# yjzxkxdn/HubertFA

Hardware: NVIDIA B200
Metric: dp_cells_per_s (higher is better)
Workload: dtype f32

## Files before the change

### hubertfa_b200/csrc/hfa_dp_skew.cu

```cuda
#include <cstdlib>

#include "hfa_common.cuh"

namespace {

__device__ __forceinline__ float sk_lds_f32(uint32_t addr)
{
    float v;
    asm volatile("ld.shared.f32 %0, [%1];" : "=f"(v) : "r"(addr));
    return v;
}
__device__ __forceinline__ float2 sk_lds_f2(uint32_t addr)
{
    float2 v;
    asm volatile("ld.shared.v2.f32 {%0, %1}, [%2];" : "=f"(v.x), "=f"(v.y) : "r"(addr));
    return v;
}
__device__ __forceinline__ void sk_sts_f32(uint32_t addr, float v)
{
    asm volatile("st.shared.f32 [%0], %1;" ::"r"(addr), "f"(v) : "memory");
}
__device__ __forceinline__ int sk_lds_i32(uint32_t addr)
{
    int v;
    asm volatile("ld.shared.s32 %0, [%1];" : "=r"(v) : "r"(addr) : "memory");
    return v;
}
__device__ __forceinline__ void sk_sts_i32(uint32_t addr, int v)
{
    asm volatile("st.shared.s32 [%0], %1;" ::"r"(addr), "r"(v) : "memory");
}
__device__ __forceinline__ void sk_mbar_init(uint32_t bar, uint32_t count)
{
    asm volatile("mbarrier.init.shared::cta.b64 [%0], %1;" ::"r"(bar), "r"(count) : "memory");
}
__device__ __forceinline__ void sk_mbar_expect_tx(uint32_t bar, uint32_t bytes)
{
    asm volatile("mbarrier.arrive.expect_tx.shared::cta.b64 _, [%0], %1;" ::"r"(bar), "r"(bytes) : "memory");
}
__device__ __forceinline__ void sk_mbar_arrive(uint32_t bar)
{
    asm volatile("mbarrier.arrive.shared::cta.b64 _, [%0];" ::"r"(bar) : "memory");
}
__device__ __forceinline__ void sk_mbar_wait(uint32_t bar, uint32_t parity)
{
    uint32_t spins = 0;
    for (;;) {
        uint32_t ok;
        asm volatile(
            "{\n"
            ".reg .pred p;\n"
            "mbarrier.try_wait.parity.shared::cta.b64 p, [%1], %2;\n"
            "selp.u32 %0, 1, 0, p;\n"
            "}\n"
            : "=r"(ok)
            : "r"(bar), "r"(parity)
            : "memory");
        if (ok) return;
        if (++spins > (1u << 24)) __trap();
    }
}
__device__ __forceinline__ void sk_bulk_load(uint32_t dst, const void *src, uint32_t bytes, uint32_t bar)
{
    asm volatile("cp.async.bulk.shared::cta.global.mbarrier::complete_tx::bytes [%0], [%1], %2, [%3];" ::"r"(dst),
                 "l"(src), "r"(bytes), "r"(bar)
                 : "memory");
}
__device__ __forceinline__ void sk_tensor_load_2d(uint32_t dst, const void *tmap, int x, int y, uint32_t bar)
{
    asm volatile(
        "cp.async.bulk.tensor.2d.shared::cta.global.tile.mbarrier::complete_tx::bytes [%0], [%1, {%2, %3}], [%4];" ::"r"(dst),
        "l"(tmap), "r"(x), "r"(y), "r"(bar)
        : "memory");
}
__device__ __forceinline__ void sk_bulk_store(void *dst, uint32_t src, uint32_t bytes)
{
    asm volatile("cp.async.bulk.global.shared::cta.bulk_group [%0], [%1], %2;" ::"l"(dst), "r"(src), "r"(bytes) : "memory");
}
__device__ __forceinline__ bool sk_elect_one()
{
    uint32_t pred;
    asm volatile(
        "{\n"
        ".reg .pred p;\n"
        "elect.sync _|p, 0xffffffff;\n"
        "selp.u32 %0, 1, 0, p;\n"
        "}\n"
        : "=r"(pred));
    return pred != 0;
}
__device__ __forceinline__ void sk_bulk_wait_read_1() { asm volatile("cp.async.bulk.wait_group.read 1;" ::: "memory"); }

__device__ __forceinline__ ulonglong2 sk_ld_slot(const ulonglong2 *p)
{
    ulonglong2 v;
    asm volatile("ld.relaxed.gpu.global.v2.u64 {%0, %1}, [%2];" : "=l"(v.x), "=l"(v.y) : "l"(p) : "memory");
    return v;
}
__device__ __forceinline__ void sk_st_slot(ulonglong2 *p, unsigned long long a, unsigned long long b)
{
    asm volatile("st.relaxed.gpu.global.v2.u64 [%0], {%1, %2};" ::"l"(p), "l"(a), "l"(b) : "memory");
}
__device__ __forceinline__ void sk_st_word(unsigned long long *p, unsigned long long a)
{
    asm volatile("st.relaxed.gpu.global.u64 [%0], %1;" ::"l"(p), "l"(a) : "memory");
}
__device__ __forceinline__ unsigned long long sk_pack(float v, uint32_t tag)
{
    return (unsigned long long)__float_as_uint(v) | ((unsigned long long)tag << 32);
}

__device__ __forceinline__ void sk_select(float up1, float stay, float up2, double pe, uint32_t sp_hi, uint32_t mr,
                                          float &dp, double &P, uint32_t &acc)
{
    asm("{\n\t"
        ".reg .pred q1, q2, q3;\n\t"
        ".reg .f32 m;\n\t"
        ".reg .f64 pn;\n\t"
        ".reg .b32 lo, hi;\n\t"
        "setp.gt.f32 q1, %3, %4;\n\t"
        "max.f32 m, %4, %3;\n\t"
        "setp.gt.f32 q2, %5, m;\n\t"
        "max.f32 %0, m, %5;\n\t"
        "@q1 lop3.b32 %2, %2, %8, 0x0000ffff, 0xf8;\n\t"
        "@q2 lop3.b32 %2, %2, %8, 0xffff0000, 0xf8;\n\t"
        "or.pred q3, q1, q2;\n\t"
        "setp.gt.or.f64 q3, %6, %1, q3;\n\t"
        "selp.f64 pn, %6, %1, q3;\n\t"
        "mov.b64 {lo, hi}, pn;\n\t"
        "and.b32 hi, hi, %7;\n\t"
        "mov.b64 %1, {lo, hi};\n\t"
        "}"
        : "=&f"(dp), "+d"(P), "+r"(acc)
        : "f"(up1), "f"(stay), "f"(up2), "d"(pe), "r"(sp_hi), "r"(mr));
}
__device__ __forceinline__ void sk_select_guarded(float up1, float stay, float up2, double pe, uint32_t sp_hi,
                                                  uint32_t mr, int live, float &dp, double &P, uint32_t &acc)
{
    asm("{\n\t"
        ".reg .pred pl, q1, q2, q3;\n\t"
        ".reg .f32 m, dn;\n\t"
        ".reg .f64 pn;\n\t"
        ".reg .b32 lo, hi, msk;\n\t"
        "setp.ne.b32 pl, %9, 0;\n\t"
        "setp.gt.and.f32 q1, %3, %4, pl;\n\t"
        "max.f32 m, %4, %3;\n\t"
        "setp.gt.and.f32 q2, %5, m, pl;\n\t"
        "max.f32 dn, m, %5;\n\t"
        "selp.f32 %0, dn, %0, pl;\n\t"
        "@q1 lop3.b32 %2, %2, %8, 0x0000ffff, 0xf8;\n\t"
        "@q2 lop3.b32 %2, %2, %8, 0xffff0000, 0xf8;\n\t"
        "or.pred q3, q1, q2;\n\t"
        "setp.gt.or.f64 q3, %6, %1, q3;\n\t"
        "and.pred q3, q3, pl;\n\t"
        "selp.f64 pn, %6, %1, q3;\n\t"
        "mov.b64 {lo, hi}, pn;\n\t"
        "selp.b32 msk, %7, 0xffffffff, pl;\n\t"
        "and.b32 hi, hi, msk;\n\t"
        "mov.b64 %1, {lo, hi};\n\t"
        "}"
        : "+f"(dp), "+d"(P), "+r"(acc)
        : "f"(up1), "f"(stay), "f"(up2), "d"(pe), "r"(sp_hi), "r"(mr), "r"(live));
}

constexpr int SK_BOXW = HFA_SKEW_BOX;
constexpr int BLK = HFA_SKEW_BLK;
constexpr uint32_t SK_ROW_B = SK_BOXW * 4u;
constexpr uint32_t SK_STG_B = BLK * SK_ROW_B;
constexpr uint32_t SK_EDGE_B = BLK * 8u;
constexpr uint32_t SK_DPST_B = BLK * 128u;
constexpr uint32_t SK_PUB_B = (2 * BLK + BLK + 32) * 4u;
constexpr int SK_LOOK = 3;
static_assert(BLK == 16 || BLK == 32, "a block is one or two backpointer words long");

template <int NSTG> struct SkSmem {
    static constexpr uint32_t TILE = 0;
    static constexpr uint32_t EDGE = TILE + (NSTG + 1) * SK_STG_B;
    static constexpr uint32_t DPST = EDGE + (NSTG + 1) * SK_EDGE_B;
    static constexpr uint32_t PUB = DPST + 2 * SK_DPST_B;
    static constexpr uint32_t FULL = PUB + 2 * SK_PUB_B;
    static constexpr uint32_t SLOT = FULL + NSTG * 8;
    static constexpr uint32_t BYTES = SLOT + 16;
};

template <int D, int NSTG, bool KEEP, bool DUMP>
__global__ void __launch_bounds__(32)
hfa_dp_skew_kernel(HfaWs ws, int item_begin, int32_t *ticket, float *__restrict__ dp_dump, int force_slow)
{
    using SM = SkSmem<NSTG>;
    constexpr int R = NSTG * BLK;
    constexpr int Q = (31 * D + BLK - 1) / BLK;
    constexpr int PF = NSTG - 1 - Q;
    static_assert(D >= 2, "advance scores must be at least two iterations old when they are consumed");
    static_assert(PF >= 1, "ring too small for this skew");
    extern __shared__ __align__(128) unsigned char smem_raw[];
    uint32_t sm0;
    {
        const uint32_t a = hfa_smem_u32(smem_raw);
        asm volatile("mov.u32 %0, %1;" : "=r"(sm0) : "r"(a));
    }

    const int lane = threadIdx.x;
    if (lane == 0) {
        sk_sts_i32(sm0 + SM::SLOT, (int)atomicInc(reinterpret_cast<unsigned int *>(ticket), gridDim.x - 1));
#pragma unroll
        for (int s = 0; s < NSTG; ++s) sk_mbar_init(sm0 + SM::FULL + 8u * s, 1);
        hfa_fence_mbar_init();
    }
    __syncwarp();
    const int item = item_begin + sk_lds_i32(sm0 + SM::SLOT);
    const HfaBandItem bi = ws.band_items[item];
    const int u = bi.utt, w = bi.band;
    const HfaUtt m = ws.utt[u];
    const int T = m.T, S = m.S, Sp = m.Sp;
    const bool has_left = w > 0, has_right = w + 1 < hfa_skew_strips(Sp);
    const int c0 = HFA_SKEW_OWN * w;
    const int s = c0 + lane;
    const bool ghost = has_left && lane < 2;
    const bool real = !ghost && s < Sp;
    const int NB = hfa_skew_blocks(D, T);
    const int n_rows = (T + 15) >> 4;
    const float2 *g_edge = ws.edge2 + m.edge_off;
    uint32_t *g_bp = ws.bp + m.bp_off;
    const unsigned char *tmap = static_cast<const unsigned char *>(ws.tmaps) + (size_t)m.tmap * 128;
    const double ratio = __ddiv_rn((double)T, (double)S);
    const float NEG = HFA_NEG_INF, POS = __uint_as_float(0x7f800000u);

    const int32_t *ids = ws.ids + m.seg_off;
    uint32_t sp_hi = 0xffffffffu;
    float jcap = NEG;
    if (s < S) {
        if (ids[s] == 0) sp_hi = 0u;
        if (s >= 2 && ids[s - 1] == 0) jcap = POS;
    }
    const bool lead_sp = (ids[0] == 0) && (S > 1);
    const bool seeded = !ghost && (s == 0 || (s == 1 && lead_sp));
    const float cap1 = (s == 0) ? NEG : POS;

    const int edge_len = (T + 15) & ~15;
    auto issue = [&](int i, int st) {
        const int t0 = i * BLK;
        const uint32_t bar = sm0 + SM::FULL + 8u * (uint32_t)st;
        if (t0 >= T) {
            sk_mbar_arrive(bar);
            return;
        }
        const uint32_t ebytes = (uint32_t)min(BLK, edge_len - t0) * 8u;
        const uint32_t bytes = SK_STG_B + ebytes;
        sk_mbar_expect_tx(bar, st == 0 ? 2u * bytes : bytes);
        sk_tensor_load_2d(sm0 + SM::TILE + (uint32_t)st * SK_STG_B, tmap, c0 & ~3, t0, bar);
        sk_bulk_load(sm0 + SM::EDGE + (uint32_t)st * SK_EDGE_B, g_edge + t0, ebytes, bar);
        if (st == 0) {
            sk_tensor_load_2d(sm0 + SM::TILE + (uint32_t)NSTG * SK_STG_B, tmap, c0 & ~3, t0, bar);
            sk_bulk_load(sm0 + SM::EDGE + (uint32_t)NSTG * SK_EDGE_B, g_edge + t0, ebytes, bar);
        }
    };
    static_assert(PF + 1 <= NSTG, "prologue fills distinct stages");
    if (sk_elect_one())
        for (int i = 0; i <= PF && i < NB; ++i) issue(i, i);
    int st_issue = (PF + 1) % NSTG;
    int st_wait = 0;
    uint32_t par_wait = 0;

    float dp = NEG;
    double P = __longlong_as_double(0xfff0000000000000ll);
    uint32_t bits = 0;
    float q1[D], q2[2 * D];
#pragma unroll
    for (int i = 0; i < D; ++i) q1[i] = NEG;
#pragma unroll
    for (int i = 0; i < 2 * D; ++i) q2[i] = NEG;

    int u_row = ((-lane * D) % R + R) % R;
    const uint32_t tile_sa = sm0 + SM::TILE + 4u * (uint32_t)(lane + (c0 & 3));
    const uint32_t edge_sa = sm0 + SM::EDGE;
    const uint32_t dpst_sa = sm0 + SM::DPST + 4u * (uint32_t)lane;
    const int o_res = (lane * D) & 15;
    const int q_rows = (lane * D + 15) >> 4;
    const uint32_t m16 = o_res ? ((0xffffu << (16 - o_res)) & 0xffffu) : 0xffffu;
    const uint32_t hi_mask = m16 | (m16 << 16);
    const uint32_t mrot0 = 0x00010001u << ((16 - o_res) & 15);
    const ulonglong2 *left_x = reinterpret_cast<const ulonglong2 *>(ws.band_xchg) +
                               (has_left ? ws.band_items[item - 1].xoff : 0);
    ulonglong2 *my_x = reinterpret_cast<ulonglong2 *>(ws.band_xchg) + bi.xoff;
    const uint32_t pub_sa = sm0 + SM::PUB +
                            ((has_right && lane == 31) ? 0u : (has_right && lane == 30) ? 4u * BLK
                                                                                        : 8u * BLK + 4u * (uint32_t)lane);
    uint32_t *bp_ptr = g_bp + (int64_t)(-q_rows) * Sp + s;
    int bp_row = -q_rows;
    float *g_dp = (KEEP && m.dp_off >= 0) ? ws.dp_store + m.dp_off + (int64_t)w * NB * (BLK * 32) : nullptr;

    ulonglong2 xv_next = make_ulonglong2(0ull, 0ull);
    auto slot_needed = [&](int jj) { const int t = BLK * jj + lane; return has_left && lane < BLK && t >= 1 && t < T; };
    if (slot_needed(0)) xv_next = sk_ld_slot(left_x + lane);

    auto flush_bits = [&](uint32_t acc, bool all_valid) {
        if (real && (all_valid || (bp_row >= 0 && bp_row < n_rows))) *bp_ptr = bits | (acc & hi_mask);
        bits = acc & ~hi_mask;
        bp_ptr += Sp;
        ++bp_row;
    };

    for (int j = 0; j < NB; ++j) {
        sk_mbar_wait(sm0 + SM::FULL + 8u * (uint32_t)st_wait, par_wait);
        const int st_cur = st_wait;
        if (++st_wait == NSTG) {
            st_wait = 0;
            par_wait ^= 1u;
        }

        if (has_left) {
            const int t = BLK * j + lane;
            const bool need = slot_needed(j);
            ulonglong2 *src = const_cast<ulonglong2 *>(left_x) + t;
            const uint32_t tag = (uint32_t)t + 1u;
            ulonglong2 v = xv_next;
            uint32_t spins = 0;
            for (;;) {
                const bool ok = !need || ((uint32_t)(v.x >> 32) == tag && (uint32_t)(v.y >> 32) == tag);
                if (__all_sync(0xffffffffu, ok)) break;
                if (++spins > (1u << 26)) __trap();
                if (!ok) v = sk_ld_slot(src);
            }
            if (slot_needed(j + 1)) xv_next = sk_ld_slot(src + BLK);
            if (lane < BLK) {
                const float a30 = need ? __uint_as_float((uint32_t)v.y) : 0.0f;
                const float a31 = need ? __uint_as_float((uint32_t)v.x) : 0.0f;
                const uint32_t row_sa = sm0 + SM::TILE + (uint32_t)st_cur * SK_STG_B + (uint32_t)lane * SK_ROW_B +
                                        4u * (uint32_t)(c0 & 3);
                sk_sts_f32(row_sa, a30);
                sk_sts_f32(row_sa + 4u, a31);
                if (st_cur == 0) {
                    sk_sts_f32(row_sa + (uint32_t)NSTG * SK_STG_B, a30);
                    sk_sts_f32(row_sa + (uint32_t)NSTG * SK_STG_B + 4u, a31);
                }
                if (need) sk_st_slot(src, 0ull, 0ull);
            }
            hfa_fence_async_smem();
            __syncwarp();
        }
        const uint32_t e_sa = tile_sa + (uint32_t)u_row * SK_ROW_B;
        const uint32_t d_sa = edge_sa + (uint32_t)u_row * 8u;
        const uint32_t k_sa = dpst_sa + (uint32_t)(j & 1) * SK_DPST_B;
        const uint32_t p_sa = pub_sa + (uint32_t)(j & 1) * SK_PUB_B;
        const bool steady = (BLK * j - 31 * D >= 1) && (BLK * j + BLK - 1 <= T - 1);

        if ((j == 0 && !has_left) || force_slow) {
            uint32_t acc = 0;
#pragma unroll 1
            for (int k = 0; k < BLK; ++k) {
                const int t = BLK * j + k - lane * D;
                const bool live = (t >= 1) && (t < T);
                const float e = sk_lds_f32(e_sa + SK_ROW_B * k);
                const float2 ed = sk_lds_f2(d_sa + 8u * k);
                const float base = __fadd_rn(dp, e);
                const float stay = __fadd_rn(base, ed.y);
                const float adv = __double2float_rn(__dadd_rn((double)__fadd_rn(base, ed.x), P));
                const float advx = ghost ? e : adv;
                const float n1 = fminf(__shfl_up_sync(0xffffffffu, advx, 1), cap1);
                const float n2 = fminf(__shfl_up_sync(0xffffffffu, advx, 2), jcap);
                const float up1 = q1[0], up2 = q2[0];
#pragma unroll
                for (int i = 0; i + 1 < D; ++i) q1[i] = q1[i + 1];
                q1[D - 1] = n1;
#pragma unroll
                for (int i = 0; i + 1 < 2 * D; ++i) q2[i] = q2[i + 1];
                q2[2 * D - 1] = n2;
                sk_sts_f32(p_sa + 4u * k, advx);
                const float mm = fmaxf(stay, up1);
                const bool b1 = up1 > stay, b2 = up2 > mm;
                const double pe = __dmul_rn((double)e, ratio);
                if (live) {
                    dp = fmaxf(mm, up2);
                    if (b1) acc |= 1u << (t & 15);
                    if (b2) acc |= 0x10000u << (t & 15);
                    const double pn = (b1 || b2 || pe > P) ? pe : P;
                    P = __hiloint2double(__double2hiint(pn) & (int)sp_hi, __double2loint(pn));
                }
                if (t == 0 && seeded) {
                    dp = e;
                    P = pe;
                }
                if (KEEP) sk_sts_f32(k_sa + 128u * k, dp);
                if (DUMP) {
                    if (!ghost && s < S && t >= 0 && t < T) dp_dump[m.cell_off + (int64_t)t * S + s] = dp;
                }
                if ((k & 15) == 15) {
                    flush_bits(acc, false);
                    acc = 0;
                }
            }
        } else {
            float ev[BLK];
            float2 dv[BLK];
#pragma unroll
            for (int k = 0; k < SK_LOOK; ++k) {
                ev[k] = sk_lds_f32(e_sa + SK_ROW_B * k);
                dv[k] = sk_lds_f2(d_sa + 8u * k);
            }
            float r1[BLK + D], r2[BLK + 2 * D];
#pragma unroll
            for (int i = 0; i < D; ++i) r1[i] = q1[i];
#pragma unroll
            for (int i = 0; i < 2 * D; ++i) r2[i] = q2[i];
            uint32_t mr = mrot0, acc = 0;
            if (!DUMP && steady) {
#pragma unroll
                for (int k = 0; k < BLK; ++k) {
                    if (k + SK_LOOK < BLK) {
                        ev[k + SK_LOOK] = sk_lds_f32(e_sa + SK_ROW_B * (k + SK_LOOK));
                        dv[k + SK_LOOK] = sk_lds_f2(d_sa + 8u * (k + SK_LOOK));
                    }
                    const float e = ev[k];
                    const float base = __fadd_rn(dp, e);
                    const float stay = __fadd_rn(base, dv[k].y);
                    const float adv = __double2float_rn(__dadd_rn((double)__fadd_rn(base, dv[k].x), P));
                    const float advx = ghost ? e : adv;
                    r1[k + D] = fminf(__shfl_up_sync(0xffffffffu, advx, 1), cap1);
                    r2[k + 2 * D] = fminf(__shfl_up_sync(0xffffffffu, advx, 2), jcap);
                    sk_sts_f32(p_sa + 4u * k, advx);
                    const double pe = __dmul_rn((double)e, ratio);
                    sk_select(r1[k], stay, r2[k], pe, sp_hi, mr, dp, P, acc);
                    mr = __funnelshift_l(mr, mr, 1);
                    if (KEEP) sk_sts_f32(k_sa + 128u * k, dp);
                    if ((k & 15) == 15) {
                        flush_bits(acc, true);
                        acc = 0;
                    }
                }
            } else {
                const int tb = BLK * j - lane * D - 1;
#pragma unroll
                for (int k = 0; k < BLK; ++k) {
                    if (k + SK_LOOK < BLK) {
                        ev[k + SK_LOOK] = sk_lds_f32(e_sa + SK_ROW_B * (k + SK_LOOK));
                        dv[k + SK_LOOK] = sk_lds_f2(d_sa + 8u * (k + SK_LOOK));
                    }
                    const int live = (unsigned)(tb + k) < (unsigned)(T - 1);
                    const float e = ev[k];
                    const float base = __fadd_rn(dp, e);
                    const float stay = __fadd_rn(base, dv[k].y);
                    const float adv = __double2float_rn(__dadd_rn((double)__fadd_rn(base, dv[k].x), P));
                    const float advx = ghost ? e : adv;
                    r1[k + D] = fminf(__shfl_up_sync(0xffffffffu, advx, 1), cap1);
                    r2[k + 2 * D] = fminf(__shfl_up_sync(0xffffffffu, advx, 2), jcap);
                    sk_sts_f32(p_sa + 4u * k, advx);
                    const double pe = __dmul_rn((double)e, ratio);
                    sk_select_guarded(r1[k], stay, r2[k], pe, sp_hi, mr, live, dp, P, acc);
                    mr = __funnelshift_l(mr, mr, 1);
                    if (KEEP) sk_sts_f32(k_sa + 128u * k, dp);
                    if (DUMP) {
                        const int t = tb + 1 + k;
                        if (!ghost && s < S && t >= 0 && t < T) dp_dump[m.cell_off + (int64_t)t * S + s] = dp;
                    }
                    if ((k & 15) == 15) {
                        flush_bits(acc, false);
                        acc = 0;
                    }
                }
            }
#pragma unroll
            for (int i = 0; i < D; ++i) q1[i] = r1[BLK + i];
#pragma unroll
            for (int i = 0; i < 2 * D; ++i) q2[i] = r2[BLK + i];
        }
        if (KEEP) hfa_fence_async_smem();
        __syncwarp();
        if (has_right) {
#pragma unroll
            for (int q = lane; q < 2 * BLK; q += 32) {
                const int half = q / BLK, i = q % BLK;
                const int t = BLK * j + i - (31 - half) * D;
                if (steady || (t >= 1 && t < T))
                    sk_st_word(reinterpret_cast<unsigned long long *>(my_x + t) + half,
                               sk_pack(sk_lds_f32(sm0 + SM::PUB + (uint32_t)(j & 1) * SK_PUB_B + 4u * (uint32_t)q),
                                       (uint32_t)t + 1u));
            }
        }
        if (sk_elect_one()) {
            if (KEEP && g_dp != nullptr) {
                sk_bulk_store(g_dp + (int64_t)j * (BLK * 32), sm0 + SM::DPST + (uint32_t)(j & 1) * SK_DPST_B, SK_DPST_B);
                hfa_bulk_commit();
                sk_bulk_wait_read_1();
            }
            if (j + PF + 1 < NB) issue(j + PF + 1, st_issue);
        }
        if (++st_issue == NSTG) st_issue = 0;
        u_row += BLK;
        if (u_row >= R) u_row -= R;
    }
    if (real && o_res != 0 && bp_row >= 0 && bp_row < n_rows) *bp_ptr = bits;
    if (!ghost) {
        if (s == S - 1) ws.dp_last[2 * u] = dp;
        if (s == S - 2) ws.dp_last[2 * u + 1] = dp;
    }
    if (KEEP && sk_elect_one()) hfa_bulk_wait_all();
}

template <int D, int NSTG, bool KEEP, bool DUMP>
cudaError_t launch_skew(const HfaLaunchCtx &c, int item_begin, int n_items, int32_t *ticket, float *dp_dump,
                        int force_slow)
{
    const size_t smem = SkSmem<NSTG>::BYTES;
    cudaError_t e = cudaFuncSetAttribute(hfa_dp_skew_kernel<D, NSTG, KEEP, DUMP>,
                                         cudaFuncAttributeMaxDynamicSharedMemorySize, (int)smem);
    if (e != cudaSuccess) return e;
    hfa_dp_skew_kernel<D, NSTG, KEEP, DUMP><<<n_items, 32, smem, c.stream>>>(c.ws, item_begin, ticket, dp_dump,
                                                                            force_slow);
    return cudaGetLastError();
}

template <int D, int NSTG>
cudaError_t launch_skew_d(const HfaLaunchCtx &c, int item_begin, int n_items, int32_t *ticket, bool keep_dp,
                          float *dp_dump, int force_slow)
{
    if (dp_dump != nullptr)
        return keep_dp ? launch_skew<D, NSTG, true, true>(c, item_begin, n_items, ticket, dp_dump, force_slow)
                       : launch_skew<D, NSTG, false, true>(c, item_begin, n_items, ticket, dp_dump, force_slow);
    return keep_dp ? launch_skew<D, NSTG, true, false>(c, item_begin, n_items, ticket, dp_dump, force_slow)
                   : launch_skew<D, NSTG, false, false>(c, item_begin, n_items, ticket, dp_dump, force_slow);
}

}

cudaError_t hfa_launch_dp_skew(const HfaLaunchCtx &c, int d, int item_begin, int n_items, int32_t *ticket,
                               bool keep_dp, float *dp_dump)
{
    if (n_items <= 0) return cudaSuccess;
    if (c.ws.tmaps == nullptr) return cudaErrorNotSupported;
    const char *sl = getenv("HFA_SKEW_SLOW");
    const int force_slow = (sl && sl[0] == '1') ? 1 : 0;
    constexpr int NS = HFA_SKEW_BLK == 32 ? 5 : 12;
    if (d == 2) return launch_skew_d<2, NS>(c, item_begin, n_items, ticket, keep_dp, dp_dump, force_slow);
    if (d == 3) return launch_skew_d<3, NS>(c, item_begin, n_items, ticket, keep_dp, dp_dump, force_slow);
    return cudaErrorInvalidValue;
}
```

Measured before the change: 84.63 billion.

## Split DP skew kernel into producer and consumer warps with mbarrier handoff

Adds a second warp per block that handles TMA issue, the left-neighbour exchange polling, publishing of boundary scores to the right band, and bulk stores of DP tiles. The compute warp now only waits on a READY barrier and signals DONE, with publish/store buffers tripled so the producer can lag. This aims to take the serialized exchange spin and store and issue latency off the DP critical path. In exchange it doubles the threads per block and adds barrier traffic, and the warp-slot parity trick used to pick the producer role is fragile.

Measured after the change: 87.57 billion, median of 6. +3.5%, better.

```diff
diff --git a/hubertfa_b200/csrc/hfa_dp_skew.cu b/hubertfa_b200/csrc/hfa_dp_skew.cu
--- a/hubertfa_b200/csrc/hfa_dp_skew.cu
+++ b/hubertfa_b200/csrc/hfa_dp_skew.cu
@@ -42,7 +42,7 @@
 {
     asm volatile("mbarrier.arrive.shared::cta.b64 _, [%0];" ::"r"(bar) : "memory");
 }
-__device__ __forceinline__ void sk_mbar_wait(uint32_t bar, uint32_t parity)
+__device__ __forceinline__ void sk_mbar_wait(uint32_t bar, uint32_t parity, uint32_t limit)
 {
     uint32_t spins = 0;
     for (;;) {
@@ -57,8 +57,22 @@
             : "r"(bar), "r"(parity)
             : "memory");
         if (ok) return;
-        if (++spins > (1u << 24)) __trap();
+        if (++spins > limit) __trap();
     }
+}
+__device__ __forceinline__ bool sk_mbar_test(uint32_t bar, uint32_t parity)
+{
+    uint32_t ok;
+    asm volatile(
+        "{\n"
+        ".reg .pred p;\n"
+        "mbarrier.test_wait.parity.shared::cta.b64 p, [%1], %2;\n"
+        "selp.u32 %0, 1, 0, p;\n"
+        "}\n"
+        : "=r"(ok)
+        : "r"(bar), "r"(parity)
+        : "memory");
+    return ok != 0;
 }
 __device__ __forceinline__ void sk_bulk_load(uint32_t dst, const void *src, uint32_t bytes, uint32_t bar)
 {
@@ -90,6 +104,7 @@
     return pred != 0;
 }
 __device__ __forceinline__ void sk_bulk_wait_read_1() { asm volatile("cp.async.bulk.wait_group.read 1;" ::: "memory"); }
+__device__ __forceinline__ void sk_bulk_wait_read_0() { asm volatile("cp.async.bulk.wait_group.read 0;" ::: "memory"); }
 
 __device__ __forceinline__ ulonglong2 sk_ld_slot(const ulonglong2 *p)
 {
@@ -171,20 +186,23 @@
 constexpr uint32_t SK_DPST_B = BLK * 128u;
 constexpr uint32_t SK_PUB_B = (2 * BLK + BLK + 32) * 4u;
 constexpr int SK_LOOK = 3;
+constexpr int SK_NBUF = 3;
 static_assert(BLK == 16 || BLK == 32, "a block is one or two backpointer words long");
 
 template <int NSTG> struct SkSmem {
     static constexpr uint32_t TILE = 0;
     static constexpr uint32_t EDGE = TILE + (NSTG + 1) * SK_STG_B;
     static constexpr uint32_t DPST = EDGE + (NSTG + 1) * SK_EDGE_B;
-    static constexpr uint32_t PUB = DPST + 2 * SK_DPST_B;
-    static constexpr uint32_t FULL = PUB + 2 * SK_PUB_B;
-    static constexpr uint32_t SLOT = FULL + NSTG * 8;
+    static constexpr uint32_t PUB = DPST + SK_NBUF * SK_DPST_B;
+    static constexpr uint32_t FULL = PUB + SK_NBUF * SK_PUB_B;
+    static constexpr uint32_t READY = FULL + NSTG * 8;
+    static constexpr uint32_t DONE = READY + NSTG * 8;
+    static constexpr uint32_t SLOT = DONE + NSTG * 8;
     static constexpr uint32_t BYTES = SLOT + 16;
 };
 
 template <int D, int NSTG, bool KEEP, bool DUMP>
-__global__ void __launch_bounds__(32)
+__global__ void __launch_bounds__(64)
 hfa_dp_skew_kernel(HfaWs ws, int item_begin, int32_t *ticket, float *__restrict__ dp_dump, int force_slow)
 {
     using SM = SkSmem<NSTG>;
@@ -200,14 +218,23 @@
         asm volatile("mov.u32 %0, %1;" : "=r"(sm0) : "r"(a));
     }
 
-    const int lane = threadIdx.x;
-    if (lane == 0) {
+    if (threadIdx.x == 0) {
+        unsigned hw_slot;
+        asm volatile("mov.u32 %0, %%warpid;" : "=r"(hw_slot));
+        sk_sts_i32(sm0 + SM::SLOT + 4u, (int)((hw_slot >> 2) & 1u));
         sk_sts_i32(sm0 + SM::SLOT, (int)atomicInc(reinterpret_cast<unsigned int *>(ticket), gridDim.x - 1));
 #pragma unroll
-        for (int s = 0; s < NSTG; ++s) sk_mbar_init(sm0 + SM::FULL + 8u * s, 1);
+        for (int s = 0; s < NSTG; ++s) {
+            sk_mbar_init(sm0 + SM::FULL + 8u * s, 1);
+            sk_mbar_init(sm0 + SM::READY + 8u * s, 32);
+            sk_mbar_init(sm0 + SM::DONE + 8u * s, 32);
+        }
         hfa_fence_mbar_init();
     }
-    __syncwarp();
+    __syncthreads();
+    const int lane = threadIdx.x & 31;
+    const bool producer =
+        __shfl_sync(0xffffffffu, (threadIdx.x >> 5) ^ (unsigned)sk_lds_i32(sm0 + SM::SLOT + 4u), 0) != 0;
     const int item = item_begin + sk_lds_i32(sm0 + SM::SLOT);
     const HfaBandItem bi = ws.band_items[item];
     const int u = bi.utt, w = bi.band;
@@ -215,14 +242,135 @@
     const int T = m.T, S = m.S, Sp = m.Sp;
     const bool has_left = w > 0, has_right = w + 1 < hfa_skew_strips(Sp);
     const int c0 = HFA_SKEW_OWN * w;
+    const int NB = hfa_skew_blocks(D, T);
+
+    if (producer) {
+        const float2 *g_edge = ws.edge2 + m.edge_off;
+        const unsigned char *tmap = static_cast<const unsigned char *>(ws.tmaps) + (size_t)m.tmap * 128;
+        float *g_dp = (KEEP && m.dp_off >= 0) ? ws.dp_store + m.dp_off + (int64_t)w * NB * (BLK * 32) : nullptr;
+        const int edge_len = (T + 15) & ~15;
+        auto issue = [&](int i, int st) {
+            const int t0 = i * BLK;
+            const uint32_t bar = sm0 + SM::FULL + 8u * (uint32_t)st;
+            if (t0 >= T) {
+                sk_mbar_arrive(bar);
+                return;
+            }
+            const uint32_t ebytes = (uint32_t)min(BLK, edge_len - t0) * 8u;
+            const uint32_t bytes = SK_STG_B + ebytes;
+            sk_mbar_expect_tx(bar, st == 0 ? 2u * bytes : bytes);
+            sk_tensor_load_2d(sm0 + SM::TILE + (uint32_t)st * SK_STG_B, tmap, c0 & ~3, t0, bar);
+            sk_bulk_load(sm0 + SM::EDGE + (uint32_t)st * SK_EDGE_B, g_edge + t0, ebytes, bar);
+            if (st == 0) {
+                sk_tensor_load_2d(sm0 + SM::TILE + (uint32_t)NSTG * SK_STG_B, tmap, c0 & ~3, t0, bar);
+                sk_bulk_load(sm0 + SM::EDGE + (uint32_t)NSTG * SK_EDGE_B, g_edge + t0, ebytes, bar);
+            }
+        };
+        static_assert(PF + 1 <= NSTG, "prologue fills distinct stages");
+        if (sk_elect_one())
+            for (int i = 0; i <= PF && i < NB; ++i) issue(i, i);
+
+        const ulonglong2 *left_x = reinterpret_cast<const ulonglong2 *>(ws.band_xchg) +
+                                   (has_left ? ws.band_items[item - 1].xoff : 0);
+        ulonglong2 *my_x = reinterpret_cast<ulonglong2 *>(ws.band_xchg) + bi.xoff;
+        auto slot_needed = [&](int jj) { const int t = BLK * jj + lane; return has_left && lane < BLK && t >= 1 && t < T; };
+        ulonglong2 xv = make_ulonglong2(0ull, 0ull);
+        if (slot_needed(0)) xv = sk_ld_slot(left_x + lane);
+
+        int a = 0, st_a = 0, buf_b = 0;
+        uint32_t par_a = 0;
+        int b = 0, st_b = 0;
+        uint32_t par_b = 0;
+        int st_issue = (PF + 1) % NSTG;
+        uint32_t spins = 0;
+        while (b < NB) {
+            if (b < a && __all_sync(0xffffffffu, sk_mbar_test(sm0 + SM::DONE + 8u * (uint32_t)st_b, par_b))) {
+                if (has_right) {
+#pragma unroll
+                    for (int q = lane; q < 2 * BLK; q += 32) {
+                        const int half = q / BLK, i = q % BLK;
+                        const int t = BLK * b + i - (31 - half) * D;
+                        if (t >= 1 && t < T)
+                            sk_st_word(reinterpret_cast<unsigned long long *>(my_x + t) + half,
+                                       sk_pack(sk_lds_f32(sm0 + SM::PUB + (uint32_t)buf_b * SK_PUB_B + 4u * (uint32_t)q),
+                                               (uint32_t)t + 1u));
+                    }
+                }
+                if (sk_elect_one()) {
+                    if (KEEP && g_dp != nullptr) {
+                        sk_bulk_store(g_dp + (int64_t)b * (BLK * 32), sm0 + SM::DPST + (uint32_t)buf_b * SK_DPST_B,
+                                      SK_DPST_B);
+                        hfa_bulk_commit();
+                    }
+                    if (b + PF + 1 < NB) issue(b + PF + 1, st_issue);
+                }
+                if (++st_issue == NSTG) st_issue = 0;
+                if (++st_b == NSTG) {
+                    st_b = 0;
+                    par_b ^= 1u;
+                }
+                if (++buf_b == SK_NBUF) buf_b = 0;
+                ++b;
+                spins = 0;
+                continue;
+            }
+            if (a < NB && a <= b + SK_NBUF - 1 &&
+                __all_sync(0xffffffffu, sk_mbar_test(sm0 + SM::FULL + 8u * (uint32_t)st_a, par_a))) {
+                bool go = true;
+                if (has_left) {
+                    const int t = BLK * a + lane;
+                    const bool need = slot_needed(a);
+                    ulonglong2 *src = const_cast<ulonglong2 *>(left_x) + t;
+                    const uint32_t tag = (uint32_t)t + 1u;
+                    const bool ok = !need || ((uint32_t)(xv.x >> 32) == tag && (uint32_t)(xv.y >> 32) == tag);
+                    go = __all_sync(0xffffffffu, ok);
+                    if (!go) {
+                        if (!ok) xv = sk_ld_slot(src);
+                    } else {
+                        const ulonglong2 v = xv;
+                        xv = slot_needed(a + 1) ? sk_ld_slot(src + BLK) : make_ulonglong2(0ull, 0ull);
+                        if (lane < BLK) {
+                            const float a30 = need ? __uint_as_float((uint32_t)v.y) : 0.0f;
+                            const float a31 = need ? __uint_as_float((uint32_t)v.x) : 0.0f;
+                            const uint32_t row_sa = sm0 + SM::TILE + (uint32_t)st_a * SK_STG_B + (uint32_t)lane * SK_ROW_B +
+                                                    4u * (uint32_t)(c0 & 3);
+                            sk_sts_f32(row_sa, a30);
+                            sk_sts_f32(row_sa + 4u, a31);
+                            if (st_a == 0) {
+                                sk_sts_f32(row_sa + (uint32_t)NSTG * SK_STG_B, a30);
+                                sk_sts_f32(row_sa + (uint32_t)NSTG * SK_STG_B + 4u, a31);
+                            }
+                            if (need) sk_st_slot(src, 0ull, 0ull);
+                        }
+                        hfa_fence_async_smem();
+                    }
+                }
+                if (go) {
+                    if (KEEP && a >= SK_NBUF && sk_elect_one()) {
+                        if (a == b + SK_NBUF - 1) sk_bulk_wait_read_0();
+                        else sk_bulk_wait_read_1();
+                    }
+                    sk_mbar_arrive(sm0 + SM::READY + 8u * (uint32_t)st_a);
+                    if (++st_a == NSTG) {
+                        st_a = 0;
+                        par_a ^= 1u;
+                    }
+                    ++a;
+                    spins = 0;
+                    continue;
+                }
+            }
+            if (++spins > (1u << 26)) __trap();
+        }
+        if (KEEP && sk_elect_one()) hfa_bulk_wait_all();
+        return;
+    }
+
     const int s = c0 + lane;
     const bool ghost = has_left && lane < 2;
     const bool real = !ghost && s < Sp;
-    const int NB = hfa_skew_blocks(D, T);
     const int n_rows = (T + 15) >> 4;
-    const float2 *g_edge = ws.edge2 + m.edge_off;
     uint32_t *g_bp = ws.bp + m.bp_off;
-    const unsigned char *tmap = static_cast<const unsigned char *>(ws.tmaps) + (size_t)m.tmap * 128;
     const double ratio = __ddiv_rn((double)T, (double)S);
     const float NEG = HFA_NEG_INF, POS = __uint_as_float(0x7f800000u);
 
@@ -237,30 +385,9 @@
     const bool seeded = !ghost && (s == 0 || (s == 1 && lead_sp));
     const float cap1 = (s == 0) ? NEG : POS;
 
-    const int edge_len = (T + 15) & ~15;
-    auto issue = [&](int i, int st) {
-        const int t0 = i * BLK;
-        const uint32_t bar = sm0 + SM::FULL + 8u * (uint32_t)st;
-        if (t0 >= T) {
-            sk_mbar_arrive(bar);
-            return;
-        }
-        const uint32_t ebytes = (uint32_t)min(BLK, edge_len - t0) * 8u;
-        const uint32_t bytes = SK_STG_B + ebytes;
-        sk_mbar_expect_tx(bar, st == 0 ? 2u * bytes : bytes);
-        sk_tensor_load_2d(sm0 + SM::TILE + (uint32_t)st * SK_STG_B, tmap, c0 & ~3, t0, bar);
-        sk_bulk_load(sm0 + SM::EDGE + (uint32_t)st * SK_EDGE_B, g_edge + t0, ebytes, bar);
-        if (st == 0) {
-            sk_tensor_load_2d(sm0 + SM::TILE + (uint32_t)NSTG * SK_STG_B, tmap, c0 & ~3, t0, bar);
-            sk_bulk_load(sm0 + SM::EDGE + (uint32_t)NSTG * SK_EDGE_B, g_edge + t0, ebytes, bar);
-        }
-    };
-    static_assert(PF + 1 <= NSTG, "prologue fills distinct stages");
-    if (sk_elect_one())
-        for (int i = 0; i <= PF && i < NB; ++i) issue(i, i);
-    int st_issue = (PF + 1) % NSTG;
     int st_wait = 0;
     uint32_t par_wait = 0;
+    int buf = 0;
 
     float dp = NEG;
     double P = __longlong_as_double(0xfff0000000000000ll);
@@ -280,19 +407,11 @@
     const uint32_t m16 = o_res ? ((0xffffu << (16 - o_res)) & 0xffffu) : 0xffffu;
     const uint32_t hi_mask = m16 | (m16 << 16);
     const uint32_t mrot0 = 0x00010001u << ((16 - o_res) & 15);
-    const ulonglong2 *left_x = reinterpret_cast<const ulonglong2 *>(ws.band_xchg) +
-                               (has_left ? ws.band_items[item - 1].xoff : 0);
-    ulonglong2 *my_x = reinterpret_cast<ulonglong2 *>(ws.band_xchg) + bi.xoff;
     const uint32_t pub_sa = sm0 + SM::PUB +
                             ((has_right && lane == 31) ? 0u : (has_right && lane == 30) ? 4u * BLK
                                                                                         : 8u * BLK + 4u * (uint32_t)lane);
     uint32_t *bp_ptr = g_bp + (int64_t)(-q_rows) * Sp + s;
     int bp_row = -q_rows;
-    float *g_dp = (KEEP && m.dp_off >= 0) ? ws.dp_store + m.dp_off + (int64_t)w * NB * (BLK * 32) : nullptr;
-
-    ulonglong2 xv_next = make_ulonglong2(0ull, 0ull);
-    auto slot_needed = [&](int jj) { const int t = BLK * jj + lane; return has_left && lane < BLK && t >= 1 && t < T; };
-    if (slot_needed(0)) xv_next = sk_ld_slot(left_x + lane);
 
     auto flush_bits = [&](uint32_t acc, bool all_valid) {
         if (real && (all_valid || (bp_row >= 0 && bp_row < n_rows))) *bp_ptr = bits | (acc & hi_mask);
@@ -302,47 +421,17 @@
     };
 
     for (int j = 0; j < NB; ++j) {
-        sk_mbar_wait(sm0 + SM::FULL + 8u * (uint32_t)st_wait, par_wait);
+        sk_mbar_wait(sm0 + SM::READY + 8u * (uint32_t)st_wait, par_wait, 1u << 26);
         const int st_cur = st_wait;
         if (++st_wait == NSTG) {
             st_wait = 0;
             par_wait ^= 1u;
         }
 
-        if (has_left) {
-            const int t = BLK * j + lane;
-            const bool need = slot_needed(j);
-            ulonglong2 *src = const_cast<ulonglong2 *>(left_x) + t;
-            const uint32_t tag = (uint32_t)t + 1u;
-            ulonglong2 v = xv_next;
-            uint32_t spins = 0;
-            for (;;) {
-                const bool ok = !need || ((uint32_t)(v.x >> 32) == tag && (uint32_t)(v.y >> 32) == tag);
-                if (__all_sync(0xffffffffu, ok)) break;
-                if (++spins > (1u << 26)) __trap();
-                if (!ok) v = sk_ld_slot(src);
-            }
-            if (slot_needed(j + 1)) xv_next = sk_ld_slot(src + BLK);
-            if (lane < BLK) {
-                const float a30 = need ? __uint_as_float((uint32_t)v.y) : 0.0f;
-                const float a31 = need ? __uint_as_float((uint32_t)v.x) : 0.0f;
-                const uint32_t row_sa = sm0 + SM::TILE + (uint32_t)st_cur * SK_STG_B + (uint32_t)lane * SK_ROW_B +
-                                        4u * (uint32_t)(c0 & 3);
-                sk_sts_f32(row_sa, a30);
-                sk_sts_f32(row_sa + 4u, a31);
-                if (st_cur == 0) {
-                    sk_sts_f32(row_sa + (uint32_t)NSTG * SK_STG_B, a30);
-                    sk_sts_f32(row_sa + (uint32_t)NSTG * SK_STG_B + 4u, a31);
-                }
-                if (need) sk_st_slot(src, 0ull, 0ull);
-            }
-            hfa_fence_async_smem();
-            __syncwarp();
-        }
         const uint32_t e_sa = tile_sa + (uint32_t)u_row * SK_ROW_B;
         const uint32_t d_sa = edge_sa + (uint32_t)u_row * 8u;
-        const uint32_t k_sa = dpst_sa + (uint32_t)(j & 1) * SK_DPST_B;
-        const uint32_t p_sa = pub_sa + (uint32_t)(j & 1) * SK_PUB_B;
+        const uint32_t k_sa = dpst_sa + (uint32_t)buf * SK_DPST_B;
+        const uint32_t p_sa = pub_sa + (uint32_t)buf * SK_PUB_B;
         const bool steady = (BLK * j - 31 * D >= 1) && (BLK * j + BLK - 1 <= T - 1);
 
         if ((j == 0 && !has_left) || force_slow) {
@@ -465,27 +554,8 @@
             for (int i = 0; i < 2 * D; ++i) q2[i] = r2[BLK + i];
         }
         if (KEEP) hfa_fence_async_smem();
-        __syncwarp();
-        if (has_right) {
-#pragma unroll
-            for (int q = lane; q < 2 * BLK; q += 32) {
-                const int half = q / BLK, i = q % BLK;
-                const int t = BLK * j + i - (31 - half) * D;
-                if (steady || (t >= 1 && t < T))
-                    sk_st_word(reinterpret_cast<unsigned long long *>(my_x + t) + half,
-                               sk_pack(sk_lds_f32(sm0 + SM::PUB + (uint32_t)(j & 1) * SK_PUB_B + 4u * (uint32_t)q),
-                                       (uint32_t)t + 1u));
-            }
-        }
-        if (sk_elect_one()) {
-            if (KEEP && g_dp != nullptr) {
-                sk_bulk_store(g_dp + (int64_t)j * (BLK * 32), sm0 + SM::DPST + (uint32_t)(j & 1) * SK_DPST_B, SK_DPST_B);
-                hfa_bulk_commit();
-                sk_bulk_wait_read_1();
-            }
-            if (j + PF + 1 < NB) issue(j + PF + 1, st_issue);
-        }
-        if (++st_issue == NSTG) st_issue = 0;
+        sk_mbar_arrive(sm0 + SM::DONE + 8u * (uint32_t)st_cur);
+        if (++buf == SK_NBUF) buf = 0;
         u_row += BLK;
         if (u_row >= R) u_row -= R;
     }
@@ -494,7 +564,6 @@
         if (s == S - 1) ws.dp_last[2 * u] = dp;
         if (s == S - 2) ws.dp_last[2 * u + 1] = dp;
     }
-    if (KEEP && sk_elect_one()) hfa_bulk_wait_all();
 }
 
 template <int D, int NSTG, bool KEEP, bool DUMP>
@@ -505,7 +574,7 @@
     cudaError_t e = cudaFuncSetAttribute(hfa_dp_skew_kernel<D, NSTG, KEEP, DUMP>,
                                          cudaFuncAttributeMaxDynamicSharedMemorySize, (int)smem);
     if (e != cudaSuccess) return e;
-    hfa_dp_skew_kernel<D, NSTG, KEEP, DUMP><<<n_items, 32, smem, c.stream>>>(c.ws, item_begin, ticket, dp_dump,
+    hfa_dp_skew_kernel<D, NSTG, KEEP, DUMP><<<n_items, 64, smem, c.stream>>>(c.ws, item_begin, ticket, dp_dump,
                                                                             force_slow);
     return cudaGetLastError();
 }
```
